# drdeford/FlipComplexityEmpirical

Hardware: AMD Instinct MI355X
Metric: flip steps/sec (whole node), 100×100 grid k=4 batched chains; % HBM peak (higher is better)
Workload: dtype int32

## Files before the change

### flipcomplexityempirical_amd/csrc/fw_grid16.hip

```cpp
#include <hip/hip_runtime.h>

#include <cstdio>
#include <cstdlib>

#include <algorithm>

#include "fw_device.h"
#include "fw_weights_bytes.h"
#include "fw_window_rows.h"

#ifdef FW_STAMPS
__device__ unsigned long long g_stamps[16];
__device__ unsigned long long g_unit_t[2 * 65536];
__device__ unsigned long long g_unit_hw[65536];
#define UNIT_TIME(u, e)                                                         \
  do {                                                                          \
    uint64_t t_;                                                                \
    asm volatile("s_memrealtime %0\n\ts_waitcnt lgkmcnt(0)" : "=s"(t_)::"memory"); \
    if (__lane_id() == 0 && (u) < 65536) {                                      \
      g_unit_t[2 * (u) + (e)] = t_;                                             \
      if ((e) == 0)                                                             \
        g_unit_hw[u] = (unsigned long long)__builtin_amdgcn_s_getreg((31 << 11) | 4) | \
                       ((unsigned long long)__builtin_amdgcn_s_getreg((31 << 11) | 20) << 32); \
    }                                                                           \
  } while (0)
#define STAMP_DECL uint64_t st_acc[16] = {}; uint64_t st_t0 = 0;
#define STAMP(i)                                              \
  do {                                                        \
    __builtin_amdgcn_sched_barrier(0);                        \
    uint64_t st_t1;                                           \
    asm volatile("s_memtime %0\n\ts_waitcnt lgkmcnt(0)" : "=s"(st_t1)::"memory"); \
    __builtin_amdgcn_sched_barrier(0);                        \
    if (i >= 0) st_acc[(i) < 0 ? 0 : (i)] += st_t1 - st_t0;   \
    st_t0 = st_t1;                                            \
  } while (0)
#define STAMP_FLUSH                                           \
  if (__lane_id() == 0)                                       \
    for (int i_ = 0; i_ < 16; ++i_) atomicAdd(&g_stamps[i_], (unsigned long long)st_acc[i_]);
#define STAMP_COUNT(i, v) st_acc[i] += (uint64_t)(v)
#else
#define STAMP_COUNT(i, v)
#define STAMP_DECL
#define STAMP(i)
#define STAMP_FLUSH
#define UNIT_TIME(u, e)
#endif

#include <cstddef>

static_assert(sizeof(fw_chain_stats) == 136, "fw_chain_stats layout");
static_assert(offsetof(fw_chain_stats, yields) == 88 && offsetof(fw_chain_stats, sum_invb) == 112 &&
                  offsetof(fw_chain_stats, cut) == 120 && offsetof(fw_chain_stats, npairs) == 128,
              "fw_chain_stats layout");

#define HIST_ADD(ptr, v) atomicAdd(ptr, v)

void* fw_grid16_pick_lean(int lb, int mode, int G, bool w4);
void* fw_grid16_pick_w2(int mode, int G, bool w4);

namespace {

constexpr int ROW = 16;
constexpr int MAX_NW = 4;
constexpr uint32_t SCR_BLOCK = 15;
constexpr int LDS_GUARD = 16;

struct Hood16 {
  int x;
  uint32_t lx;
  uint32_t bits;
  uint32_t cnt;
  bool has_v;
  int deg;
};

struct GDiv {
  uint32_t m, s;
  __device__ __forceinline__ int operator()(int x) const {
    return (int)(__umul24((uint32_t)x, m) >> s);
  }
};
__device__ __forceinline__ int mulW(int r, int W) { return (int)__umul24((uint32_t)r, (uint32_t)W); }

__device__ __forceinline__ uint32_t rowbits(uint64_t bal, int row) {
  return (uint32_t)(bal >> (row * ROW)) & 0xFFFFu;
}
__device__ __forceinline__ uint32_t row_scan(uint32_t x) {
  x += (uint32_t)__builtin_amdgcn_update_dpp(0, (int)x, 0x111, 0xF, 0xF, true);
  x += (uint32_t)__builtin_amdgcn_update_dpp(0, (int)x, 0x112, 0xF, 0xF, true);
  x += (uint32_t)__builtin_amdgcn_update_dpp(0, (int)x, 0x114, 0xF, 0xF, true);
  x += (uint32_t)__builtin_amdgcn_update_dpp(0, (int)x, 0x118, 0xF, 0xF, true);
  return x;
}
__device__ __forceinline__ uint32_t row_last(uint32_t x) {
  return (uint32_t)__builtin_amdgcn_update_dpp(0, (int)x, 0x15F, 0xF, 0xF, false);
}
__device__ __forceinline__ uint32_t row_sum(uint32_t x) { return row_last(row_scan(x)); }
__device__ __forceinline__ uint32_t row_first(uint32_t x) {
  return (uint32_t)__builtin_amdgcn_update_dpp(0, (int)x, 0x150, 0xF, 0xF, false);
}
__device__ __forceinline__ uint32_t row_shl1(uint32_t x) {
  return (uint32_t)__builtin_amdgcn_update_dpp(0, (int)x, 0x101, 0xF, 0xF, false);
}
__device__ __forceinline__ uint32_t row_pick(uint32_t x, int L, int q) {
  const int src = ((__lane_id() - q) + L) << 2;
  return (uint32_t)__builtin_amdgcn_ds_bpermute(src, (int)x);
}

template <int LB>
__device__ __forceinline__ uint32_t lab_window(const LDS uint8_t* lab, int x) {
  const int bit = (x - 1) * LB;
  const int wi = bit >> 5;
  const LDS uint32_t* w = reinterpret_cast<const LDS uint32_t*>(lab);
  const uint32_t lo0 = w[wi];
  const uint32_t lo = wi >= 0 ? lo0 : 0u;
  const uint32_t hi = w[wi + 1];
  const uint64_t both = ((uint64_t)hi << 32) | lo;
  return (uint32_t)(both >> (uint32_t)(bit - wi * 32)) & ((1u << (6 * LB)) - 1u);
}

template <int LB, int MODE>
__device__ __forceinline__ void weights4(const LDS uint8_t* lab, int x0, int W, int H, int n,
                                         GDiv gd, uint32_t& w4, uint32_t& cd4) {
  constexpr uint32_t M = (1u << LB) - 1u;
  w4 = 0;
  cd4 = 0;
  if (x0 >= n) return;
  const uint32_t own = lab_window<LB>(lab, x0);
  const uint32_t up = x0 + 3 - W >= 0 ? lab_window<LB>(lab, x0 - W) : 0u;
  const uint32_t dn = x0 + W < n ? lab_window<LB>(lab, x0 + W) : 0u;
  const int r0 = gd(x0);
  const int c0 = x0 - mulW(r0, W);
#pragma unroll
  for (int tt = 0; tt < 4; ++tt) {
    int ct = c0 + tt, rt = r0;
    if (ct >= W) {
      ct -= W;
      rt += 1;
    }
    const uint32_t lx = (own >> (LB * (tt + 1))) & M;
    const uint32_t ll = (own >> (LB * tt)) & M;
    const uint32_t lr = (own >> (LB * (tt + 2))) & M;
    const uint32_t lu = (up >> (LB * (tt + 1))) & M, ld = (dn >> (LB * (tt + 1))) & M;
    uint32_t bits = 0, cd = 0;
    if (rt > 0) { bits |= 1u << lu; cd += lu != lx; }
    if (ct > 0) { bits |= 1u << ll; cd += ll != lx; }
    if (ct < W - 1) { bits |= 1u << lr; cd += lr != lx; }
    if (rt < H - 1) { bits |= 1u << ld; cd += ld != lx; }
    uint32_t w = MODE == FW_PROPOSE_CUTEDGE ? cd : (uint32_t)__popc(bits & ~(1u << lx));
    if (x0 + tt >= n) w = cd = 0;
    w4 |= w << (8 * tt);
    cd4 |= cd << (8 * tt);
  }
}

__device__ __forceinline__ uint32_t bsum4(uint32_t v) {
  return (v & 0xFFu) + ((v >> 8) & 0xFFu) + ((v >> 16) & 0xFFu) + (v >> 24);
}

__device__ __forceinline__ uint32_t spread4(uint32_t u) {
  const uint32_t t = ((u << 12) | u) & 0x000F000Fu;
// ... 209 lines not shown
        else
          V |= nw;
      }
    }
  }
  if (verdict < 0) return -1;
  const uint32_t pc = (uint32_t)__popc(P);
  uint32_t dg = pc * (uint32_t)((r > 0) + (r < H - 1) + 2);
  if (c0 <= 0) dg -= (P >> (-c0)) & 1u;
  if (hi_n <= 32) dg -= (P >> (hi_n - 1)) & 1u;
  nodes = row_sum(pc);
  degs = row_sum(dg);
  return verdict;
}

__device__ __forceinline__ uint32_t lane_read(uint32_t x, int L) {
  return (uint32_t)__builtin_amdgcn_ds_bpermute(L << 2, (int)x);
}
template <int R>
__device__ __forceinline__ uint32_t grp_sum(uint32_t x, int gb, int q) {
  uint32_t t = 0;
#pragma unroll
  for (int s = 0; s < R; ++s) t += lane_read(x, gb + s * ROW + q);
  return t;
}
template <int R>
__device__ __forceinline__ uint64_t grp_sum64(uint64_t x, int gb, int q) {
  uint64_t t = 0;
#pragma unroll
  for (int s = 0; s < R; ++s)
    t += (uint64_t)lane_read((uint32_t)x, gb + s * ROW + q) |
         ((uint64_t)lane_read((uint32_t)(x >> 32), gb + s * ROW + q) << 32);
  return t;
}

__device__ __forceinline__ void scr_clear(LDS uint8_t* scr, int x) {
  __atomic_fetch_and(PK<4>::word(scr, x), ~(15u << PK<4>::shift(x)), __ATOMIC_RELAXED);
}

template <int LB>
__device__ bool grid_race(const LDS uint8_t* lab, LDS uint8_t* scr, LDS uint32_t* list,
                          GLB uint32_t* spill, int qcap, int W, int H, GDiv gd, int lane,
                          int v, uint32_t a, int m, int src, uint64_t cls, uint64_t& bfs_nodes,
                          uint64_t& bfs_deg) {
  using P = PK<LB>;
  using S = PK<4>;
  auto list_get = [&](int i) -> uint32_t {
    const uint32_t in_lds = list[i < qcap ? i : qcap - 1];
    uint32_t in_hbm = 0;
    if (i >= qcap) in_hbm = spill[i - qcap];
    return i < qcap ? in_lds : in_hbm;
  };
  auto list_put = [&](int i, uint32_t x) {
    if (i < qcap) list[i] = x;
    if (i >= qcap) spill[i - qcap] = x;
  };
  if (lane == 0) S::axor(scr, v, SCR_BLOCK);
  if (lane < m) {
    S::axor(scr, src, 1u + (uint32_t)lane);
    list_put(lane, (uint32_t)src);
  }
  lds_order();
  int nl = m, lb = 0, le = m;
  uint32_t my_deg = 0;
  int verdict = -1;
  for (;;) {
    uint64_t rep = ballot(lane < m && (__ffsll((unsigned long long)cls) - 1) == lane);
    if (__popcll(rep) == 1) {
      verdict = 1;
      break;
    }
    uint64_t pushed_src = 0;
    for (int base = lb; base < le; base += WAVE) {
      const int idx = base + lane;
      const bool act = idx < le;
      const int x = act ? (int)list_get(idx) : 0;
      const uint32_t o = act ? S::get(scr, x) - 1u : 0u;
      const int xr = gd(x);
      const int xc = x - mulW(xr, W);
      if (act) my_deg += (uint32_t)((xr > 0) + (xc > 0) + (xc < W - 1) + (xr < H - 1));
      bfs_nodes += (uint64_t)__popcll(ballot(act));
#pragma unroll
      for (int j = 0; j < 4; ++j) {
        int y = -1;
        if (act) {
          if (j == 0 && xr > 0) y = x - W;
          if (j == 1 && xc > 0) y = x - 1;
          if (j == 2 && xc < W - 1) y = x + 1;
          if (j == 3 && xr < H - 1) y = x + W;
        }
        bool push = false, req = false;
        uint32_t other = 0;
        if (y >= 0 && P::get(lab, y) == a) {
          const uint32_t got = S::claim(scr, y, 0u, 1u + o);
          if (got == 0u) {
            push = true;
          } else if (got - 1u < (uint32_t)m) {
            req = true;
            other = got - 1u;
          }
        }
        const uint64_t pm = ballot(push);
        if (push) list_put(nl + (int)mbcnt(pm), (uint32_t)y);
        nl += __popcll(pm);
        if (pm) {
          for (int si = 0; si < m; ++si)
            pushed_src |= ballot(push && o == (uint32_t)si) ? (1ull << si) : 0ull;
        }
        uint64_t rm = ballot(req && o != other);
        while (rm) {
          const int Lr = __ffsll((unsigned long long)rm) - 1;
          rm &= rm - 1;
          const int o1 = rdl((int32_t)o, Lr), o2 = rdl((int32_t)other, Lr);
          const uint64_t m1 = rdl64(cls, o1), m2 = rdl64(cls, o2);
          if (m1 != m2) {
            const uint64_t nm = m1 | m2;
            if (lane < m && ((nm >> lane) & 1ull)) cls = nm;
          }
        }
      }
      if (nl > qcap) __threadfence_block();
    }
    lds_order();
    lb = le;
    le = nl;
    rep = ballot(lane < m && (__ffsll((unsigned long long)cls) - 1) == lane);
    if (__popcll(rep) == 1) {
      verdict = 1;
      break;
    }
    const bool closed = lane < m && ((rep >> lane) & 1ull) && ((cls & pushed_src) == 0ull);
    if (ballot(closed)) {
      verdict = 0;
      break;
    }
  }
  bfs_deg += wave_sum(my_deg);
  for (int base = 0; base < nl; base += WAVE) {
    const int idx = base + lane;
    if (idx < nl) scr_clear(scr, (int)list_get(idx));
  }
  if (lane == 0) scr_clear(scr, v);
  lds_order();
  return verdict == 1;
}

template <int LB, int MODE, int PER, bool FULL, bool BIG, int R, bool W2 = false, bool W4 = false>
__device__ __forceinline__ void grid16_body(const FwRunParams& p) {
  static_assert(!W4 || LB == 2, "the width flag belongs to the SWAR weights");
  static_assert(PER % 2 == 0, "group sums are read as u16 pairs");
  static_assert(R == 1 || R == 2 || R == 4, "rows per chain");
  static_assert(R == 1 || (!FULL && !BIG), "speculation: lean small-grid kernels only");
  constexpr int CPW = 4 / R;
  extern __shared__ __align__(16) uint8_t smem[];
  __shared__ int32_t s_lock;
  using P = PK<LB>;
  const int lane = __lane_id(), row = lane >> 4, q = lane & 15;
  const int sx = row & (R - 1);
  const int grp = row / R;
  const int gb = grp * R * ROW;
  const bool owner = sx == 0;
  const int wv = (int)(threadIdx.x >> 6);
  const int W = (int)in_vgpr((uint32_t)p.g.gw), H = (int)in_vgpr((uint32_t)p.g.gh);
  const int n = (int)in_vgpr((uint32_t)p.g.n);
  const int D = (int)in_vgpr((uint32_t)p.g.maxdeg), G = (int)in_vgpr((uint32_t)p.G);
  const int k = (int)in_vgpr((uint32_t)p.k);
  LDS uint8_t* const sm = (LDS uint8_t*)smem;
  LDS uint8_t* const lab = sm + LDS_GUARD + (wv * CPW + grp) * p.slot_stride;
  LDS uint32_t* const gsum = reinterpret_cast<LDS uint32_t*>(lab + p.off_gsum);
  LDS uint32_t* const ssum = reinterpret_cast<LDS uint32_t*>(lab + p.off_ssum);
  LDS uint32_t* const lvl1 = BIG ? ssum : gsum;
  LDS uint8_t* const scr = sm + p.off_scr;
  LDS uint32_t* const list = reinterpret_cast<LDS uint32_t*>(sm + p.off_list16);
  GLB uint32_t* const spill = (GLB uint32_t*)(p.spill + (size_t)blockIdx.x * (size_t)n);
  const uint32_t key0 = (uint32_t)p.seed, key1 = (uint32_t)(p.seed >> 32);
  const int GW = (G + 1) >> 1;
  const int SG = (G + 15) >> 4;
  const bool maps_on = FULL && p.m_acc != nullptr;
  const int32_t pop_lo = (int32_t)in_vgpr((uint32_t)(int32_t)max(p.pop_lo, (int64_t)INT32_MIN));
  const int32_t pop_hi = (int32_t)in_vgpr((uint32_t)(int32_t)min(p.pop_hi, (int64_t)INT32_MAX));
  const GDiv gd{in_vgpr(p.g.gm24), in_vgpr(p.g.gs24)};
  const int32_t rule = FULL ? p.accept : FW_ACCEPT_CUT;
  int my_dr, my_dc;
  role_off(q <= 8 ? q : 0, my_dr, my_dc);
  if (LB == 2 && q >= 9 && q <= 12) {
    my_dr = q == 9 ? -2 : (q == 12 ? 2 : 0);
    my_dc = q == 10 ? -2 : (q == 11 ? 2 : 0);
  }
  const uint32_t nb_lanes = q == 0   ? 0x1Eu
                            : q == 1 ? (1u << 9) | (1u << 8) | (1u << 5)
                            : q == 2 ? (1u << 10) | (1u << 8) | (1u << 7)
                            : q == 3 ? (1u << 11) | (1u << 5) | (1u << 6)
                            : q == 4 ? (1u << 12) | (1u << 6) | (1u << 7)
                                     : 0u;
  auto divmod = [&](int x, int& r, int& c) {
    r = gd(x);
    c = x - mulW(r, W);
  };
  STAMP_DECL

  {
    LDS uint32_t* s32 = reinterpret_cast<LDS uint32_t*>(scr);
    for (int i = (int)threadIdx.x; i < p.scr_bytes / 4; i += (int)blockDim.x) s32[i] = 0u;
    if (threadIdx.x == 0) s_lock = 0;
  }
  __syncthreads();

  const int nq = (p.n_chains + CPW - 1) / CPW;
  for (;;) {
    int cb = 0;
    if (lane == 0) cb = atomicAdd(p.next_chain, 1);
    const int u = rdl(cb, 0);
    if (u >= nq * p.slices) break;
    const int seg = u / nq;
    const int quad = u - seg * nq;
    const uint32_t ustep = (uint32_t)(p.steps * (seg + 1) / p.slices - p.steps * seg / p.slices);
    if (seg > 0) {
      for (;;) {
        const int done =
            rfl(__hip_atomic_load(p.seg_done + quad, __ATOMIC_RELAXED, __HIP_MEMORY_SCOPE_AGENT));
        if (done >= seg) break;
        __builtin_amdgcn_s_sleep(2);
      }
      __builtin_amdgcn_fence(__ATOMIC_ACQUIRE, "agent");
    }
    UNIT_TIME(u, 0);
    const int cbase = quad * CPW;
    const int c = cbase + grp;
    const bool has = c < p.n_chains;
    const int cc = has ? c : cbase;
    const uint64_t gid = (uint64_t)(p.chain_id0 + c);
    const bool cached = p.gcache_ok != 0 || seg > 0;

    constexpr bool OPQ = R > 1 || MODE == FW_PROPOSE_CUTEDGE;
    int ql = q;
    if constexpr (OPQ) asm volatile("" : "+v"(ql));
    {
      const u32x4* src = reinterpret_cast<const u32x4*>(p.labels + (size_t)cc * p.lab_stride);
      LDS u32x4* dst = reinterpret_cast<LDS u32x4*>(lab);
      const int nv = cached ? p.lab_copy16 : p.lab_bytes / 16;
      for (int i = sx * ROW + ql; i < nv; i += R * ROW) dst[i] = src[i];
    }
    int32_t pops = ql < k ? (int32_t)p.pops[(size_t)cc * k + ql] : 0;
    double thr_l = FULL && ql < 2 * D + 1 ? p.thr[(size_t)cc * p.thr_stride + ql] : 0.0;
    uint64_t thr53_l = ql < 2 * D + 1 ? p.thr53[(size_t)cc * p.thr_stride + ql] : 0ull;
    fw_chain_stats* stp = p.stats + cc;
    const uint64_t acc0 = FULL && p.sched ? stp->accepts : 0ull;
    auto sched_row = [&](uint64_t nacc) {
      const int64_t t = (int64_t)(acc0 + nacc) + 1 - p.sched_t0;
      const int64_t r = t < 0 ? 0 : (t >= p.sched_rows ? p.sched_rows - 1 : t);
      if (q < 2 * D + 1) {
        thr_l = p.sched[r * (2 * D + 1) + q];
        thr53_l = p.sched53[r * (2 * D + 1) + q];
      }
    };
    if (FULL && p.sched) sched_row(0);
    uint64_t att0 = stp->attempts;
    const bool first = has && !stp->stuck && stp->yields == 0 && att0 == 0;
    uint32_t n_att = 0;
    const uint64_t yields0 = stp->yields;
    int32_t stuck = has ? stp->stuck : 1;
    uint32_t s_cut = 0, s_bn = 0;
    double sum_invb = stp->sum_invb;
    const bool waits_on = FULL && p.wsamp != nullptr;
    double wsum = waits_on ? p.wsamp[2 * (size_t)cc] : 0.0;
    double wcur = waits_on ? p.wsamp[2 * (size_t)cc + 1] : 0.0;
    uint32_t n_steps = 0, n_acc = 0, n_popf = 0, n_conf = 0, n_sdeg = 0, n_adeg = 0, n_bchg = 0;
    uint32_t retries = 0;
    uint64_t n_bfs = 0, n_bfsn = 0, n_bfsd = 0;
    uint32_t bpos_w = ROW * R;
    Pend pend = maps_on ? pend_load(p, cc) : Pend{-1, 0, 0u};
    int32_t bcnt = rule == FW_ACCEPT_BOUNDARY && ql < k ? p.bcnt[(size_t)cc * k + ql] : 0;
    lds_order();

    int32_t cut, bnodes, npairs;
    {
      uint32_t cut2 = 0, bn = 0, np = 0;
      for (int t2 = 0; t2 < (cached ? 0 : GW); ++t2) {
        uint32_t tot[2];
#pragma unroll
        for (int h = 0; h < 2; ++h) {
          uint32_t w4, cd4;
          weights4x<LB, MODE, true, true, W4>(lab, 2 * t2 + h, q, W, H, n, gd, w4, cd4);
          const uint32_t ws = bsum4m(w4);
          cut2 += bsum4m(cd4);
          bn += ((cd4 & 0xFFu) != 0) + ((cd4 & 0xFF00u) != 0) + ((cd4 & 0xFF0000u) != 0) +
                ((cd4 & 0xFF000000u) != 0);
          np += ws;
          tot[h] = row_sum(ws);
        }
        if (q == 0 && has) gsum[t2] = tot[0] | (tot[1] << 16);
      }
      if constexpr (BIG) {
        for (int t2 = GW + q; t2 < SG * 8; t2 += ROW)
          if (has) gsum[t2] = 0u;
        lds_order();
        for (int w2 = q; w2 < 8 * PER; w2 += ROW) {
          uint32_t s2[2] = {0u, 0u};
#pragma unroll
          for (int h = 0; h < 2; ++h) {
            const int sg = 2 * w2 + h;
            if (sg < SG)
              for (int i = 0; i < 8; ++i) {
                const uint32_t g2 = gsum[sg * 8 + i];
                s2[h] += (g2 & 0xFFFFu) + (g2 >> 16);
              }
          }
          if (has) ssum[w2] = s2[0] | (s2[1] << 16);
        }
      } else {
        for (int t2 = GW + q; t2 < 8 * PER; t2 += ROW)
          if (has) gsum[t2] = 0u;
      }
      if (cached) {
        cut = stp->cut;
        bnodes = stp->bnodes;
        npairs = stp->npairs;
      } else {
        cut = (int32_t)(row_sum(cut2) / 2);
        bnodes = (int32_t)row_sum(bn);
        npairs = (int32_t)row_sum(np);
      }
    }
    lds_order();
    double invb = p.g.invb[bnodes];

    const int RN = FULL ? p.ring_n : 0;
    auto ring_pair = [&]() -> int32_t {
      int f = -1, sc = -1;
      for (int b0 = 0; b0 < RN; b0 += ROW) {
        const int r = b0 + q;
        const int ri = r < RN ? r : 0;
        uint32_t m = rowbits(ballot(r < RN && P::get(lab, p.ring_u[ri]) != P::get(lab, p.ring_w[ri])),
                             row);
        if (m && f < 0) {
          f = b0 + __ffs(m) - 1;
          m &= m - 1;
        }
        if (m && sc < 0) sc = b0 + __ffs(m) - 1;
      }
      return sc >= 0 ? f * RN + sc : RN * RN;
    };
    int32_t rpair = RN && has ? ring_pair() : 0;
    uint32_t rrun = 0;

    uint32_t hc0 = 0, hc1 = 0, hb0 = 0, hb1 = 0;
    int32_t base_c = max(0, cut - 16), base_b = max(0, bnodes - 16);
    auto observe = [&](bool on) {
      if (!on) return;
      if (FULL) rrun += 1;
      if (waits_on) wsum += wcur;
      s_cut += (uint32_t)cut;
      s_bn += (uint32_t)bnodes;
      sum_invb += invb;
      int ic = cut - base_c;
      if (ic < 0 || ic >= 2 * ROW) {
        if (hc0) HIST_ADD(p.hist_cut + base_c + q, (unsigned long long)hc0);
        if (hc1) HIST_ADD(p.hist_cut + base_c + ROW + q, (unsigned long long)hc1);
        hc0 = hc1 = 0;
        base_c = max(0, cut - ROW);
        ic = cut - base_c;
      }
      hc0 += ic == q;
      hc1 += ic == q + ROW;
      int ib = bnodes - base_b;
      if (ib < 0 || ib >= 2 * ROW) {
        if (hb0) HIST_ADD(p.hist_b + base_b + q, (unsigned long long)hb0);
        if (hb1) HIST_ADD(p.hist_b + base_b + ROW + q, (unsigned long long)hb1);
        hb0 = hb1 = 0;
        base_b = max(0, bnodes - ROW);
        ib = bnodes - base_b;
      }
      hb0 += ib == q;
      hb1 += ib == q + ROW;
    };
    if (waits_on && first) wcur = wait_draw(p.seed, FW_WAIT_T0, gid, p.wlp[bnodes]);
    observe(first && owner);

    U4 pb = {0u, 0u, 0u, 0u};
    int bpos = ROW;
    uint32_t w2[PER / 2];
    auto read_lvl1 = [&]() {
#pragma unroll
      for (int t = 0; t < PER / 2; ++t) w2[t] = lvl1[q * (PER / 2) + t];
    };
    read_lvl1();

    const bool unit_pop = !FULL || p.g.pop == nullptr;
    const uint32_t psh = (uint32_t)p.prio_shift;
    const uint32_t pstep = ustep >= (2u << psh) ? ustep >> psh : 2u;
    uint32_t pnext = pstep, plev = 0;
    if (psh == 3u && (__builtin_amdgcn_s_getreg((3 << 11) | 4) & 1u) == 0u) plev = 1;
    if (plev == 0) __builtin_amdgcn_s_setprio(3);
    else __builtin_amdgcn_s_setprio(2);
    for (;;) {
      STAMP(-1);
      if (!stuck && (retries >= (uint32_t)p.max_retries || npairs == 0)) stuck = 1;
      const bool act = has && !stuck && n_steps < ustep;
      if (ballot(act) == 0ull) break;
      if (rfl(n_steps) >= pnext) {
        pnext += pstep;
        plev = (plev + 1u) & 3u;
        if (plev == 0) __builtin_amdgcn_s_setprio(3);
        else if (plev == 1) __builtin_amdgcn_s_setprio(2);
        else if (plev == 2) __builtin_amdgcn_s_setprio(1);
        else __builtin_amdgcn_s_setprio(0);
      }

      U4 x;
      if constexpr (R == 1) {
        if (bpos == ROW) {
          if (n_sdeg >= p.fold_at || (s_cut | s_bn) >= p.fold_at) {
            if (q == 0 && has) {
              stp->pop_fail += n_popf;
              stp->contig_fail += n_conf;
              stp->sum_deg += n_sdeg;
              stp->sum_cut += s_cut;
              stp->sum_bnodes += s_bn;
            }
            att0 += n_att;
            n_att = n_popf = n_conf = n_sdeg = 0;
            s_cut = s_bn = 0;
          }
          const uint64_t t = att0 + (uint64_t)(n_att + (uint32_t)q);
          pb = philox((uint32_t)t, (uint32_t)(t >> 32), (uint32_t)gid, (uint32_t)(gid >> 32),
                      in_vgpr(key0), in_vgpr(key1));
          bpos = 0;
        }
        x = U4{row_first(pb.x0), row_first(pb.x1), row_first(pb.x2), row_first(pb.x3)};
        pb = U4{row_shl1(pb.x0), row_shl1(pb.x1), row_shl1(pb.x2), row_shl1(pb.x3)};
        ++bpos;
        n_att += act ? 1u : 0u;
      } else {
        if (bpos_w > (uint32_t)(ROW * R - R)) {
          const uint32_t s_any = lane_read(s_cut | s_bn, gb + q);
          if (4u * n_att >= p.fold_at || s_any >= p.fold_at) {
            const uint32_t f0 = grp_sum<R>(n_popf, gb, q), f1 = grp_sum<R>(n_conf, gb, q);
            const uint32_t f2 = grp_sum<R>(n_sdeg, gb, q);
            if (q == 0 && owner && has) {
              stp->pop_fail += f0;
              stp->contig_fail += f1;
              stp->sum_deg += f2;
              stp->sum_cut += s_cut;
              stp->sum_bnodes += s_bn;
            }
            att0 += n_att;
            n_att = n_popf = n_conf = n_sdeg = 0;
            s_cut = s_bn = 0;
          }
          const uint64_t t = att0 + (uint64_t)(n_att + (uint32_t)(sx * ROW + q));
          pb = philox((uint32_t)t, (uint32_t)(t >> 32), (uint32_t)gid, (uint32_t)(gid >> 32),
                      in_vgpr(key0), in_vgpr(key1));
          bpos_w = 0;
        }
        const int srcl = gb + (int)bpos_w + sx;
        x = U4{lane_read(pb.x0, srcl), lane_read(pb.x1, srcl), lane_read(pb.x2, srcl),
               lane_read(pb.x3, srcl)};
      }
      const uint32_t r = scale64(x.x0, x.x1, (uint32_t)(npairs > 0 ? npairs : 1));

      STAMP(0);
      uint32_t s = 0;
#pragma unroll
      for (int t = 0; t < PER / 2; ++t) s += (w2[t] & 0xFFFFu) + (w2[t] >> 16);
      uint32_t pp[PER / 2];
      {
        uint32_t base = 0;
#pragma unroll
        for (int t = 0; t < PER / 2; ++t) {
          pp[t] = __umul24(base, 0x10001u) + (w2[t] + (w2[t] << 16));
          base = pp[t] >> 16;
        }
      }
      const uint32_t incl = row_scan(s);
      const uint32_t rb1 = rowbits(ballot(incl > r), row);
      const int Lw = __ffs(rb1) - 1;
      const uint32_t rl = r - (incl - s);
      typedef uint16_t u16x2 __attribute__((ext_vector_type(2)));
      const u16x2 rl2 = __builtin_bit_cast(u16x2, __umul24(rl & 0xFFFFu, 0x10001u));
      u16x2 mn = {0xFFFFu, 0xFFFFu}, wraps = {0u, 0u};
#pragma unroll
      for (int t = 0; t < PER / 2; ++t) {
        const u16x2 e = rl2 - __builtin_bit_cast(u16x2, pp[t]);
        mn = __builtin_elementwise_min(mn, e);
        wraps += e >> (uint16_t)15;
      }
      const uint32_t rem = min(rl, (uint32_t)min(mn.x, mn.y));
      const int tfu = PER - (int)wraps.x - (int)wraps.y;
      const int tf = min(tfu, PER - 1);
      const uint32_t pk1 = row_pick(((uint32_t)(q * PER + tf) << 16) | (rem & 0xFFFFu), Lw, q);
      int gi;
      uint32_t r1;
      uint32_t rbg = 1u;
      if constexpr (BIG) {
        const int sgi = min((int)(pk1 >> 16), SG - 1);
        const uint32_t r1s = pk1 & 0xFFFFu;
        const uint32_t g2 = gsum[sgi * 8 + (q >> 1)];
        const uint32_t gv = (q & 1) ? (g2 >> 16) : (g2 & 0xFFFFu);
        const uint32_t incg = row_scan(gv);
        rbg = rowbits(ballot(incg > r1s), row);
        const int Lg = __ffs(rbg) - 1;
        const uint32_t pkg =
            row_pick(((uint32_t)(sgi * 16 + q) << 16) | ((r1s - (incg - gv)) & 0xFFFFu), Lg, q);
        gi = min((int)(pkg >> 16), G - 1);
        r1 = pkg & 0xFFFFu;
      } else {
        gi = min((int)(pk1 >> 16), G - 1);
        r1 = pk1 & 0xFFFFu;
      }

      STAMP(1);
      uint32_t w4, cd4;
      weights4x<LB, MODE, false, !W2, W4>(lab, gi, q, W, H, n, gd, w4, cd4);
      const uint32_t pref1 = w4 + (w4 << 8);
      const uint32_t pref = pref1 + (pref1 << 16);
      const uint32_t ws = pref >> 24;
      const uint32_t incl2 = row_scan(ws);
      const uint32_t rb2 = rowbits(ballot(incl2 > r1), row);
      const int L2 = __ffs(rb2) - 1;
      const uint32_t r2 = min(r1 - (incl2 - ws), 127u);
      const uint32_t gt = ((pref | 0x80808080u) - __builtin_amdgcn_perm(0u, r2 + 1u, 0u)) & 0x80808080u;
      const int t2 = gt ? (__ffs(gt) - 1) >> 3 : 3;
      const uint32_t bef2 = t2 ? (pref >> (8 * t2 - 8)) & 0xFFu : 0u;
      const uint32_t pk2 = row_pick(((uint32_t)(q * 4 + t2) << 16) | ((r2 - bef2) & 0xFFFFu), L2, q);
      const int v = min(gi * 64 + (int)(pk2 >> 16), n - 1);
      const uint32_t j = pk2 & 0xFFFFu;
      if (R == 1 && act && (rb1 == 0 || rb2 == 0 || rbg == 0)) stuck = 2;
      const bool go = act && rb1 != 0 && rb2 != 0 && rbg != 0;

      STAMP(2);
      int vr, vc;
      divmod(v, vr, vc);
      const int dv = (vr > 0) + (vc > 0) + (vc < W - 1) + (vr < H - 1);
      Hood16 h;
      h.x = -1;
      h.lx = NOLAB;
      h.bits = 0;
      h.cnt = 0;
      h.has_v = false;
      h.deg = 0;
      if constexpr (LB == 2) {
        const int xr = vr + my_dr, xc = vc + my_dc;
        const bool inb = (q <= 12) & ((uint32_t)xr < (uint32_t)H) & ((uint32_t)xc < (uint32_t)W);
        const int xx = mulW(xr, W) + xc;
        const uint32_t l0 = P::get(lab, inb ? xx : v);
        h.x = inb ? xx : -1;
        h.lx = inb ? l0 : NOLAB;
        const uint32_t m0 = rowbits(ballot(h.lx == 0u), row) & nb_lanes;
        const uint32_t m1 = rowbits(ballot(h.lx == 1u), row) & nb_lanes;
        const uint32_t m2 = rowbits(ballot(h.lx == 2u), row) & nb_lanes;
        const uint32_t m3 = rowbits(ballot(h.lx == 3u), row) & nb_lanes;
        h.bits = (m0 ? 1u : 0u) | (m1 ? 2u : 0u) | (m2 ? 4u : 0u) | (m3 ? 8u : 0u);
        if constexpr (MODE == FW_PROPOSE_CUTEDGE) {
          const uint32_t same = h.lx == 0u ? m0 : h.lx == 1u ? m1 : h.lx == 2u ? m2 : m3;
          h.cnt = (uint32_t)__popc(m0 | m1 | m2 | m3) - (uint32_t)__popc(same);
          h.deg = q == 0 ? (int)h.cnt + (int)__popc(same) : 0;
        }
        h.has_v = q >= 1 && q <= 4 && inb;
        if (!(inb && q <= 4)) {
          h.bits = 0;
          h.cnt = 0;
        }
      } else {
        const int xr = vr + my_dr, xc = vc + my_dc;
        if (q <= 8 && xr >= 0 && xr < H && xc >= 0 && xc < W) {
          h.x = xr * W + xc;
          h.lx = P::get(lab, h.x);
          if (q <= 4) {
            h.deg = (xr > 0) + (xc > 0) + (xc < W - 1) + (xr < H - 1);
            const int vslot = 4 - q;
#pragma unroll
            for (int jj = 0; jj < 4; ++jj) {
              int y = -1;
              if (jj == 0 && xr > 0) y = h.x - W;
              if (jj == 1 && xc > 0) y = h.x - 1;
              if (jj == 2 && xc < W - 1) y = h.x + 1;
              if (jj == 3 && xr < H - 1) y = h.x + W;
              if (y < 0) continue;
              if (q > 0 && jj == vslot) {
                h.has_v = true;
                continue;
              }
              const uint32_t ly = P::get(lab, y);
              h.bits |= 1u << ly;
              h.cnt += ly != h.lx;
            }
          }
        }
      }
      const uint32_t a = row_first(h.lx);
      const bool isnb = q >= 1 && q <= 4 && h.x >= 0;
      uint32_t d;
      if constexpr (MODE == FW_PROPOSE_CUTEDGE) {
        const uint32_t cm = rowbits(ballot(isnb && h.lx != a), row) >> 1;
        uint32_t mm = cm;
        for (uint32_t t = 0; t < j && t < 4; ++t) mm &= mm - 1;
        const int Lc = __ffs(mm);
        d = row_pick(h.lx, Lc, q);
      } else {
        uint32_t mask;
        if constexpr (LB == 2) {
          mask = row_first(h.bits) & ~(1u << a);
        } else {
          uint32_t fb = (isnb && h.lx != a) ? (1u << h.lx) : 0u;
          fb |= (uint32_t)__builtin_amdgcn_update_dpp(0, (int)fb, 0x111, 0xF, 0xF, true);
          fb |= (uint32_t)__builtin_amdgcn_update_dpp(0, (int)fb, 0x112, 0xF, 0xF, true);
          fb |= (uint32_t)__builtin_amdgcn_update_dpp(0, (int)fb, 0x114, 0xF, 0xF, true);
          mask = (uint32_t)__builtin_amdgcn_update_dpp(0, (int)fb, 0x154, 0xF, 0xF, false);
        }
        uint32_t mm = mask;
        if constexpr (LB == 2) {
          const uint32_t m1 = mm & (mm - 1u), m2 = m1 & (m1 - 1u);
          mm = j == 0u ? mm : (j == 1u ? m1 : m2);
        } else {
          for (uint32_t t = 0; t < j && t < 15; ++t) mm &= mm - 1;
        }
        d = (uint32_t)(__ffs(mm) - 1);
      }
      const uint32_t amb = rowbits(ballot(isnb && h.lx == a), row) >> 1;
      const int m = __popc(amb);
      const int nbd = __popc(rowbits(ballot(isnb && h.lx == d), row) >> 1);
      const int dcut = m - nbd;

// ... 72 lines not shown
        uint32_t vt = win_touch(fx, q) | (win_miss(fx, ex4) ? 1u : 0u);
        vt |= (uint32_t)__builtin_amdgcn_update_dpp(0, (int)vt, 0x111, 0xF, 0xF, true);
        vt |= (uint32_t)__builtin_amdgcn_update_dpp(0, (int)vt, 0x112, 0xF, 0xF, true);
        vt |= (uint32_t)__builtin_amdgcn_update_dpp(0, (int)vt, 0x114, 0xF, 0xF, true);
        vt = (uint32_t)__builtin_amdgcn_update_dpp(0, (int)vt, 0x156, 0xF, 0xF, false);
        const int wvd = win_verdict((vt & 1u) != 0u, vt, ex4);
        STAMP_COUNT(12, 1);
        STAMP_COUNT(13, nflood);
        if (need & (wvd >= 0)) {
          contig = wvd == 1;
          need = false;
        }
      }
      STAMP(7);
      if (BIG && !p.no_bb && !p.no_rowbb && ballot(need)) {
        uint32_t bn16 = 0, bd16 = 0;
        const int vb = grid_race_bb_row<LB>(lab, n, W, H, q, row, need, vr, vc, a, amb,
                                            (uint32_t)(lNE | (lES << 1) | (lSW << 2) | (lWN << 3)),
                                            bn16, bd16);
        if (need && vb >= 0) {
          contig = vb == 1;
          need = false;
          count_search(bn16, bd16);
        }
      }
      uint64_t rows_need = ballot(q == 0 && need);
      bool locked = false;
      while (rows_need) {
        const int L0 = __ffsll((unsigned long long)rows_need) - 1;
        rows_need &= rows_need - 1;
        const int rr = L0 >> 4;
        if constexpr (R > 1) {
          if (rr % R) {
            const uint64_t sure = ballot(q == 0 && go && pop_ok && contig && wacc);
            const uint32_t before = (uint32_t)((1u << (rr % R)) - 1u) << (rr - rr % R);
            uint32_t rows_sure = 0;
#pragma unroll
            for (int r4 = 0; r4 < 4; ++r4) rows_sure |= ((sure >> (16 * r4)) & 1u) << r4;
            if (rows_sure & before) continue;
          }
        }
        const uint32_t aa = rdl(a, L0);
        const uint32_t am4 = rdl(amb, L0);
        const uint32_t lk = rdl((uint32_t)(lNE | (lES << 1) | (lSW << 2) | (lWN << 3)), L0);
        uint64_t bn = 0, bd = 0;
        int verdict = -1;
        if (!p.no_bb)
          verdict = grid_race_bb<LB>(sm + LDS_GUARD + (wv * CPW + rr / R) * p.slot_stride, n, W, H,
                                    lane, rdl(vr, L0), rdl(vc, L0), aa, am4, lk, bn, bd);
        if (verdict >= 0) {
          if (row == rr) {
            contig = verdict == 1;
            count_search(bn, bd);
          }
          continue;
        }
        if (!locked) {
          if (lane == 0) {
            int expect = 0;
            while (!__hip_atomic_compare_exchange_strong(&s_lock, &expect, 1, __ATOMIC_ACQUIRE,
                                                         __ATOMIC_RELAXED,
                                                         __HIP_MEMORY_SCOPE_WORKGROUP)) {
              expect = 0;
              __builtin_amdgcn_s_sleep(1);
            }
          }
          lds_order();
          locked = true;
        }
        const int vv = rdl(v, L0);
        const int mr = __popc(am4);
        int srcn = -1;
        uint32_t mm = am4;
        for (int i = 0; i < mr; ++i) {
          const int bit = __ffs(mm) - 1;
          mm &= mm - 1;
          const int val = rdl(h.x, L0 + 1 + bit);
          if (lane == i) srcn = val;
        }
        uint64_t cls = lane < mr ? (1ull << lane) : 0ull;
        auto sx = [&](int b) { return __popc(am4 & ((1u << b) - 1u)); };
        auto merge = [&](int s1, int s2) {
          const uint64_t nm = rdl64(cls, s1) | rdl64(cls, s2);
          if (lane < mr && ((nm >> lane) & 1ull)) cls = nm;
        };
        if (lk & 1) merge(sx(0), sx(2));
        if (lk & 2) merge(sx(2), sx(3));
        if (lk & 4) merge(sx(3), sx(1));
        if (lk & 8) merge(sx(1), sx(0));
        const bool ok = grid_race<LB>(sm + LDS_GUARD + (wv * CPW + rr / R) * p.slot_stride, scr, list, spill,
                                      p.qcap16, W, H, gd, lane, vv, aa, mr, srcn, cls, bn,
                                      bd);
        if (row == rr) {
          contig = ok;
          count_search(bn, bd);
        }
      }
      if (locked && lane == 0)
        __hip_atomic_store(&s_lock, 0, __ATOMIC_RELEASE, __HIP_MEMORY_SCOPE_WORKGROUP);

      STAMP(4);
      const bool valid = go && pop_ok && contig;
      if constexpr (R > 1) {
        const bool accepted = valid && wacc;
        const uint64_t b_go = ballot(q == 0 && go), b_val = ballot(q == 0 && valid);
        const uint64_t b_acc = ballot(q == 0 && accepted);
        uint32_t cons = 0, kold = 0, ns = n_steps, rt = retries;
        int fpos = -1;
        bool stop = !act;
#pragma unroll
        for (int s2 = 0; s2 < R; ++s2) {
          const int L = gb + s2 * ROW;
          const bool g2 = (b_go >> L) & 1ull, v2 = (b_val >> L) & 1ull, a2 = (b_acc >> L) & 1ull;
          if (!stop && !g2) {
            stuck = 2;
            stop = true;
          }
          if (!stop) {
            cons = (uint32_t)s2 + 1u;
            if (v2) {
              ns += 1u;
              rt = 0u;
              if (a2) {
                fpos = s2;
                stop = true;
              } else {
                kold += 1u;
              }
              if (ns >= ustep) stop = true;
            } else {
              rt += 1u;
              if (rt >= (uint32_t)p.max_retries) stop = true;
            }
          }
        }
        if (sx < (int)cons) {
          n_sdeg += (uint32_t)dv;
          if (!pop_ok) n_popf += 1;
          else if (!contig) n_conf += 1;
          n_bfs += it_bfs;
          n_bfsn += it_bfsn;
          n_bfsd += it_bfsd;
        }
        n_steps = ns;
        retries = rt;
        n_att += cons;
        bpos_w += cons;
        const bool commit_me = sx == fpos;
        if (commit_me) {
          n_acc += 1;
          n_adeg += (uint32_t)dv;
          n_bchg += (uint32_t)(plus + minus);
          if (q == 0) P::axor(lab, v, a ^ d);
          if (mine && wn != wo) lds_add(gsum + (h.x >> 7), (wn - wo) << (16 * ((h.x >> 6) & 1)));
        }
        lds_order();
        read_lvl1();
        uint32_t dl = commit_me && mine ? wn - wo : 0u;
        dl += (uint32_t)__builtin_amdgcn_update_dpp(0, (int)dl, 0x111, 0xF, 0xF, true);
        dl += (uint32_t)__builtin_amdgcn_update_dpp(0, (int)dl, 0x112, 0xF, 0xF, true);
        dl += (uint32_t)__builtin_amdgcn_update_dpp(0, (int)dl, 0x114, 0xF, 0xF, true);
        const int dnp = (int)(uint32_t)__builtin_amdgcn_update_dpp(0, (int)dl, 0x154, 0xF, 0xF, false);
        const int fsrc = gb + (fpos < 0 ? 0 : fpos) * ROW + q;
        const uint32_t pk = (uint32_t)(dcut + 8) | ((uint32_t)plus << 4) | ((uint32_t)minus << 8) |
                            (a << 12) | (d << 16) | ((uint32_t)(dnp + 64) << 20);
        const uint32_t pkf = lane_read(pk, fsrc);
        const uint64_t ib = (uint64_t)__double_as_longlong(invb_new);
        const uint32_t ibl = lane_read((uint32_t)ib, fsrc), ibh = lane_read((uint32_t)(ib >> 32), fsrc);
        for (uint32_t i = 0; i < kold; ++i) observe(owner);
        if (fpos >= 0) {
          npairs += (int)((pkf >> 20) & 127u) - 64;
          cut += (int)(pkf & 15u) - 8;
          bnodes += (int)((pkf >> 4) & 15u) - (int)((pkf >> 8) & 15u);
          invb = __longlong_as_double((long long)(((uint64_t)ibh << 32) | ibl));
          if ((uint32_t)q == ((pkf >> 12) & 15u)) pops -= 1;
          if ((uint32_t)q == ((pkf >> 16) & 15u)) pops += 1;
          observe(owner);
        }
        STAMP(5);
        continue;
      }
      if (go) {
        n_sdeg += (uint32_t)dv;
        if (!pop_ok) n_popf += 1;
        else if (!contig) n_conf += 1;
        retries = valid ? 0u : retries + 1u;
      }
      bool accepted;
      if (rule == FW_ACCEPT_BOUNDARY) {
        const int32_t fv = p.flags[v] ? 1 : 0;
        const int32_t cnt = bcnt - ((uint32_t)q == a ? fv : 0) + ((uint32_t)q == d ? fv : 0);
        accepted = valid && __popc(rowbits(ballot(q < k && cnt > 0), row)) >= 2;
      } else {
        bool acc_l;
        if (rule == FW_ACCEPT_BRATIO) {
          const double bound = thr_l * ((double)(bnodes + plus - minus) / (double)bnodes);
          acc_l = u53(x.x2, x.x3) < bound;
        } else {
          acc_l = (((uint64_t)(x.x2 >> 5) << 26) | (uint64_t)(x.x3 >> 6)) < thr53_l;
        }
        accepted = valid & (((rowbits(ballot(acc_l), row) >> (dcut + D)) & 1u) != 0u);
      }
      STAMP(8);
      if (FULL && p.trace != nullptr && valid && q == 0)
        p.trace[(size_t)c * p.steps + n_steps] = accepted ? v * 64 + (int)d : -1;
      n_steps += valid ? 1u : 0u;
      if (maps_on && accepted) {
        const int64_t t = (int64_t)(yields0 + (n_steps - 1u) + (first ? 1u : 0u));
        if (q >= 1 && q <= 4 && h.x >= 0 && (h.lx == a || h.lx == d)) {
          const int e = q == 1   ? grid_eid_down(vr - 1, vc, W, H)
                        : q == 2 ? grid_eid_right(vr, vc - 1, W, H)
                        : q == 3 ? grid_eid_right(vr, vc, W, H)
                                 : grid_eid_down(vr, vc, W, H);
          map_edge(p, c, e, h.lx == a, t);
        }
        if (q == 0) map_run_end(p, c, pend, t);
        pend = Pend{v, (int32_t)d, (uint32_t)t};
      }

      if (accepted) {
        if (q == 0) P::axor(lab, v, a ^ d);
        if (mine && wn != wo) {
          lds_add(gsum + (h.x >> 7), (wn - wo) << (16 * ((h.x >> 6) & 1)));
          if (BIG) lds_add(ssum + (h.x >> 11), (wn - wo) << (16 * ((h.x >> 10) & 1)));
        }
      }
      lds_order();
      read_lvl1();
      uint32_t dl = accepted && mine ? wn - wo : 0u;
      dl += (uint32_t)__builtin_amdgcn_update_dpp(0, (int)dl, 0x111, 0xF, 0xF, true);
      dl += (uint32_t)__builtin_amdgcn_update_dpp(0, (int)dl, 0x112, 0xF, 0xF, true);
      dl += (uint32_t)__builtin_amdgcn_update_dpp(0, (int)dl, 0x114, 0xF, 0xF, true);
      const int dnp = (int)(uint32_t)__builtin_amdgcn_update_dpp(0, (int)dl, 0x154, 0xF, 0xF, false);
      if (FULL && RN && accepted && p.ring_node[v]) {
        const int32_t np2 = ring_pair();
        if (np2 != rpair) {
          if (q == 0 && rrun) atomicAdd(p.hist_ring + rpair, (unsigned long long)rrun);
          rrun = 0;
          rpair = np2;
        }
      }
      STAMP(9);
      asm volatile("" ::"v"(invb_new));
      invb = accepted ? invb_new : invb;
      if (accepted) {
        n_acc += 1;
        if (FULL && p.sched) sched_row(n_acc);
        n_adeg += (uint32_t)dv;
        npairs += dnp;
        cut += dcut;
        bnodes += plus - minus;
        n_bchg += (uint32_t)(plus + minus);
        if ((uint32_t)q == a) pops -= pv;
        if ((uint32_t)q == d) pops += pv;
        if (rule == FW_ACCEPT_BOUNDARY && p.flags[v]) {
          if ((uint32_t)q == a) bcnt -= 1;
          if ((uint32_t)q == d) bcnt += 1;
        }
        if (waits_on) wcur = wait_draw(p.seed, att0 + (uint64_t)(n_att - 1u), gid, p.wlp[bnodes]);
      }
      observe(valid);
      STAMP(5);
    }

    STAMP(6);
    if constexpr (R > 1) {
      n_popf = grp_sum<R>(n_popf, gb, q);
      n_conf = grp_sum<R>(n_conf, gb, q);
      n_sdeg = grp_sum<R>(n_sdeg, gb, q);
      n_acc = grp_sum<R>(n_acc, gb, q);
      n_adeg = grp_sum<R>(n_adeg, gb, q);
      n_bchg = grp_sum<R>(n_bchg, gb, q);
      n_bfs = grp_sum64<R>(n_bfs, gb, q);
      n_bfsn = grp_sum64<R>(n_bfsn, gb, q);
      n_bfsd = grp_sum64<R>(n_bfsd, gb, q);
    }
    if (has && owner) {
      if (hc0) HIST_ADD(p.hist_cut + base_c + q, (unsigned long long)hc0);
      if (hc1) HIST_ADD(p.hist_cut + base_c + ROW + q, (unsigned long long)hc1);
      if (hb0) HIST_ADD(p.hist_b + base_b + q, (unsigned long long)hb0);
      if (hb1) HIST_ADD(p.hist_b + base_b + ROW + q, (unsigned long long)hb1);
      if (FULL && RN && q == 0 && rrun) atomicAdd(p.hist_ring + rpair, (unsigned long long)rrun);
      int qw = q;
      if constexpr (OPQ) asm volatile("" : "+v"(qw));
      u32x4* dst = reinterpret_cast<u32x4*>(p.labels + (size_t)c * p.lab_stride);
      const LDS u32x4* src = reinterpret_cast<const LDS u32x4*>(lab);
      for (int i = qw; i < p.lab_copy16; i += ROW) dst[i] = src[i];
      if (qw < k) p.pops[(size_t)c * k + qw] = (int64_t)pops;
      if (qw < k && rule == FW_ACCEPT_BOUNDARY) p.bcnt[(size_t)c * k + qw] = bcnt;
      if (q == 0 && maps_on) pend_store(p, c, pend);
      if (q == 0 && waits_on) {
        p.wsamp[2 * (size_t)c] = wsum;
        p.wsamp[2 * (size_t)c + 1] = wcur;
      }
      if (q <= 8) {
        int qr = qw;
        if constexpr (!OPQ) asm volatile("" : "+v"(qr));
        uint64_t* rec = reinterpret_cast<uint64_t*>(stp) + 2 * qr;
        const uint64_t o0 = rec[0];
        const uint64_t o1 = qr < 8 ? rec[1] : 0ull;
        const uint64_t yinc = (uint64_t)n_steps + (first ? 1u : 0u);
        uint64_t w0, w1;
        switch (q) {
          case 0: w0 = att0 + n_att; w1 = o1 + n_steps; break;
          case 1: w0 = o0 + n_acc; w1 = o1 + n_popf; break;
          case 2: w0 = o0 + n_conf; w1 = o1 + n_bfs; break;
          case 3: w0 = o0 + n_bfsn; w1 = o1 + n_bfsd; break;
          case 4: w0 = o0 + n_sdeg; w1 = o1 + n_adeg; break;
          case 5: w0 = o0 + n_bchg; w1 = o1 + yinc; break;
          case 6: w0 = o0 + s_cut; w1 = o1 + s_bn; break;
          case 7:
            w0 = (uint64_t)__double_as_longlong(sum_invb);
            w1 = (uint64_t)(uint32_t)cut | ((uint64_t)(uint32_t)bnodes << 32);
            break;
          default: w0 = (uint64_t)(uint32_t)npairs | ((uint64_t)(uint32_t)stuck << 32); w1 = 0;
        }
        if (qr < 8) {
          typedef uint64_t u64x2 __attribute__((ext_vector_type(2)));
          *reinterpret_cast<u64x2*>(rec) = u64x2{w0, w1};
        } else {
          rec[0] = w0;
        }
      }
    }
    lds_order();
    UNIT_TIME(u, 1);
    if (seg + 1 < p.slices) {
      __builtin_amdgcn_fence(__ATOMIC_RELEASE, "agent");
      __hip_atomic_store(p.seg_done + quad, seg + 1, __ATOMIC_RELAXED, __HIP_MEMORY_SCOPE_AGENT);
    }
  }
  STAMP_FLUSH
}

template <int LB, int MODE, int PER, bool FULL, bool BIG, bool W4 = false>
__global__ __launch_bounds__(64 * MAX_NW) __attribute__((amdgpu_waves_per_eu(3))) void fw_grid16_kernel(FwRunParams p) {
  static_assert(!FULL, "FULL instantiations: fw_grid16_full_kernel");
  grid16_body<LB, MODE, PER, FULL, BIG, 1, false, W4>(p);
}
template <int LB, int MODE, int PER, bool FULL, bool BIG>
__global__ __launch_bounds__(64 * MAX_NW) void fw_grid16_full_kernel(FwRunParams p) {
  grid16_body<LB, MODE, PER, true, BIG, 1>(p);
}
template <int LB, int MODE, int PER, bool W4>
__global__ __launch_bounds__(64 * MAX_NW) void fw_grid16_w2_kernel(FwRunParams p) {
  grid16_body<LB, MODE, PER, false, false, 1, true, W4>(p);
}

#ifndef FW_SPEC_WPE
#define FW_SPEC_WPE 3
#endif
template <int LB, int MODE, int PER, int R>
__global__ __launch_bounds__(64 * MAX_NW) __attribute__((amdgpu_waves_per_eu(FW_SPEC_WPE))) void
fw_grid16_spec_kernel(FwRunParams p) {
  grid16_body<LB, MODE, PER, false, false, R>(p);
}

int per16(int G) { return G <= 16 * 2 ? 2 : G <= 16 * 4 ? 4 : G <= 16 * 10 ? 10 : 16; }
int per16_big(int G) { return (G + 15) / 16 <= 32 ? 2 : 4; }
bool is_big(int G) { return G > 16 * 16; }

template <int LB, int MODE, int PER, bool FULL, bool BIG, bool W4 = false>
void* k16() {
  if constexpr (FULL)
    return reinterpret_cast<void*>(&fw_grid16_full_kernel<LB, MODE, PER, true, BIG>);
  else
    return reinterpret_cast<void*>(&fw_grid16_kernel<LB, MODE, PER, false, BIG, W4>);
}

template <int LB, int MODE, bool W4>
void* pick16_small_lean_w(int G) {
  switch (per16(G)) {
    case 2: return k16<LB, MODE, 2, false, false, W4>();
    case 4: return k16<LB, MODE, 4, false, false, W4>();
    case 10: return k16<LB, MODE, 10, false, false, W4>();
    default: return k16<LB, MODE, 16, false, false, W4>();
  }
}
template <int LB, int MODE>
void* pick16_small_lean(int G, bool w4) {
  if constexpr (LB == 2) {
    if (w4) return pick16_small_lean_w<LB, MODE, true>(G);
  }
  return pick16_small_lean_w<LB, MODE, false>(G);
}

template <int LB, int MODE, bool FULL>
void* pick16(int G, bool w4) {
  if (is_big(G)) {
    if constexpr (LB == 4) {
      return nullptr;
    } else {
      return per16_big(G) == 2
                 ? k16<LB, MODE, 2, FULL, true>()
                 : k16<LB, MODE, 4, FULL, true>();
    }
  }
  if constexpr (LB == 3) {
    return nullptr;
  } else if constexpr (FULL) {
    switch (per16(G)) {
      case 2: return k16<LB, MODE, 2, true, false>();
      case 4: return k16<LB, MODE, 4, true, false>();
      case 10: return k16<LB, MODE, 10, true, false>();
      default: return k16<LB, MODE, 16, true, false>();
    }
  } else {
#if defined(FW_STAMPS)
    return pick16_small_lean<LB, MODE>(G, w4);
#else
    return fw_grid16_pick_lean(LB, MODE, G, w4);
#endif
  }
}

template <int MODE, bool W4>
void* pick16_w2(int G) {
  if (is_big(G)) return nullptr;
  switch (per16(G)) {
    case 2: return reinterpret_cast<void*>(&fw_grid16_w2_kernel<2, MODE, 2, W4>);
    case 4: return reinterpret_cast<void*>(&fw_grid16_w2_kernel<2, MODE, 4, W4>);
    case 10: return reinterpret_cast<void*>(&fw_grid16_w2_kernel<2, MODE, 10, W4>);
    default: return reinterpret_cast<void*>(&fw_grid16_w2_kernel<2, MODE, 16, W4>);
  }
}

template <int LB, int MODE, int R>
void* pick16_spec(int G) {
  if (is_big(G) || LB == 3) return nullptr;
  switch (per16(G)) {
// ... 266 lines not shown
```

Baseline: 4.644 billion.

## Store level-1 weight sums as in-lane prefix sums to skip per-step scan

For small non-W2 kernels, the level-1 group-sum array in LDS now holds per-lane inclusive prefix sums instead of raw pair sums. Each step can read the lane total and prefixes directly, with no per-step summation and prefix loop. Weight updates now add the delta to every word from the changed position to the end of the lane's span, which means several LDS atomics instead of one. The array is converted back to raw sums before the final write-out.

After: 4.655 billion, median of 6. Within noise of the previous version (+0.2%).

```diff
diff --git a/flipcomplexityempirical_amd/csrc/fw_grid16.hip b/flipcomplexityempirical_amd/csrc/fw_grid16.hip
--- a/flipcomplexityempirical_amd/csrc/fw_grid16.hip
+++ b/flipcomplexityempirical_amd/csrc/fw_grid16.hip
@@ -7,6 +7,7 @@
 
 #include "fw_device.h"
 #include "fw_weights_bytes.h"
+#include "fw_lvl1_prefix.h"
 #include "fw_window_rows.h"
 
 #ifdef FW_STAMPS
@@ -522,6 +523,7 @@
   static_assert(R == 1 || R == 2 || R == 4, "rows per chain");
   static_assert(R == 1 || (!FULL && !BIG), "speculation: lean small-grid kernels only");
   constexpr int CPW = 4 / R;
+  constexpr bool L1P = !BIG && !W2;
   extern __shared__ __align__(16) uint8_t smem[];
   __shared__ int32_t s_lock;
   using P = PK<LB>;
@@ -693,6 +695,17 @@
       }
     }
     lds_order();
+    if constexpr (L1P) {
+      if (owner) {
+        uint32_t base = 0;
+#pragma unroll
+        for (int t = 0; t < PER / 2; ++t) {
+          LDS uint32_t* const wp = gsum + q * (PER / 2) + t;
+          *wp = l1_prefix_word(*wp, base);
+        }
+      }
+      lds_order();
+    }
     double invb = p.g.invb[bnodes];
 
     const int RN = FULL ? p.ring_n : 0;
@@ -749,12 +762,26 @@
 
     U4 pb = {0u, 0u, 0u, 0u};
     int bpos = ROW;
-    uint32_t w2[PER / 2];
+    uint32_t pp[PER / 2];
     auto read_lvl1 = [&]() {
 #pragma unroll
-      for (int t = 0; t < PER / 2; ++t) w2[t] = lvl1[q * (PER / 2) + t];
+      for (int t = 0; t < PER / 2; ++t) pp[t] = lvl1[q * (PER / 2) + t];
     };
     read_lvl1();
+    auto lvl1_commit = [&](int x, uint32_t dlt) {
+      if constexpr (!L1P) {
+        lds_add(gsum + (x >> 7), dlt << (16 * ((x >> 6) & 1)));
+        if (BIG) lds_add(ssum + (x >> 11), dlt << (16 * ((x >> 10) & 1)));
+      } else {
+        int jw, cnt;
+        l1_commit_span<PER / 2>(x, jw, cnt);
+        LDS uint32_t* const wp = gsum + jw;
+        lds_add(wp, l1_commit_addend(dlt, x, 0));
+#pragma unroll
+        for (int t = 1; t < PER / 2; ++t)
+          if (t < cnt) lds_add(wp + t, l1_commit_addend(dlt, x, t));
+      }
+    };
 
     const bool unit_pop = !FULL || p.g.pop == nullptr;
     const uint32_t psh = (uint32_t)p.prio_shift;
@@ -830,15 +857,17 @@
       const uint32_t r = scale64(x.x0, x.x1, (uint32_t)(npairs > 0 ? npairs : 1));
 
       STAMP(0);
-      uint32_t s = 0;
-#pragma unroll
-      for (int t = 0; t < PER / 2; ++t) s += (w2[t] & 0xFFFFu) + (w2[t] >> 16);
-      uint32_t pp[PER / 2];
-      {
+      uint32_t s;
+      if constexpr (L1P) {
+        s = pp[PER / 2 - 1] >> 16;
+      } else {
+        s = 0;
+#pragma unroll
+        for (int t = 0; t < PER / 2; ++t) s += (pp[t] & 0xFFFFu) + (pp[t] >> 16);
         uint32_t base = 0;
 #pragma unroll
         for (int t = 0; t < PER / 2; ++t) {
-          pp[t] = __umul24(base, 0x10001u) + (w2[t] + (w2[t] << 16));
+          pp[t] = __umul24(base, 0x10001u) + (pp[t] + (pp[t] << 16));
           base = pp[t] >> 16;
         }
       }
@@ -1217,7 +1246,7 @@
           n_adeg += (uint32_t)dv;
           n_bchg += (uint32_t)(plus + minus);
           if (q == 0) P::axor(lab, v, a ^ d);
-          if (mine && wn != wo) lds_add(gsum + (h.x >> 7), (wn - wo) << (16 * ((h.x >> 6) & 1)));
+          if (mine && wn != wo) lvl1_commit(h.x, wn - wo);
         }
         lds_order();
         read_lvl1();
@@ -1285,10 +1314,7 @@
 
       if (accepted) {
         if (q == 0) P::axor(lab, v, a ^ d);
-        if (mine && wn != wo) {
-          lds_add(gsum + (h.x >> 7), (wn - wo) << (16 * ((h.x >> 6) & 1)));
-          if (BIG) lds_add(ssum + (h.x >> 11), (wn - wo) << (16 * ((h.x >> 10) & 1)));
-        }
+        if (mine && wn != wo) lvl1_commit(h.x, wn - wo);
       }
       lds_order();
       read_lvl1();
@@ -1341,6 +1367,15 @@
       n_bfsd = grp_sum64<R>(n_bfsd, gb, q);
     }
     if (has && owner) {
+      if constexpr (L1P) {
+        uint32_t base = 0;
+#pragma unroll
+        for (int t = 0; t < PER / 2; ++t) {
+          LDS uint32_t* const wp = gsum + q * (PER / 2) + t;
+          *wp = l1_sums_word(*wp, base);
+        }
+        lds_order();
+      }
       if (hc0) HIST_ADD(p.hist_cut + base_c + q, (unsigned long long)hc0);
       if (hc1) HIST_ADD(p.hist_cut + base_c + ROW + q, (unsigned long long)hc1);
       if (hb0) HIST_ADD(p.hist_b + base_b + q, (unsigned long long)hb0);
diff --git a/flipcomplexityempirical_amd/csrc/fw_lvl1_prefix.h b/flipcomplexityempirical_amd/csrc/fw_lvl1_prefix.h
--- /dev/null
+++ b/flipcomplexityempirical_amd/csrc/fw_lvl1_prefix.h
@@ -0,0 +1,36 @@
+#pragma once
+#include <stdint.h>
+
+#if defined(__HIPCC__) || defined(__CUDACC__)
+#define FW_L1_FN __host__ __device__ inline
+#else
+#define FW_L1_FN inline
+#endif
+
+FW_L1_FN uint32_t l1_prefix_word(uint32_t sums, uint32_t& base) {
+  const uint32_t t = base + sums;
+  const uint32_t pp = t + (t << 16);
+  base = pp >> 16;
+  return pp;
+}
+
+FW_L1_FN uint32_t l1_sums_word(uint32_t prefixes, uint32_t& base) {
+  const uint32_t lo = prefixes & 0xFFFFu, hi = prefixes >> 16;
+  const uint32_t sums = ((lo - base) & 0xFFFFu) | ((hi - lo) << 16);
+  base = hi;
+  return sums;
+}
+
+template <int PER2>
+FW_L1_FN void l1_commit_span(int x, int& jw, int& cnt) {
+  static_assert(PER2 == 1 || PER2 == 2 || PER2 == 5 || PER2 == 8, "PER in {2, 4, 10, 16}");
+  constexpr uint32_t M = (1024u + PER2 - 1) / PER2;
+  jw = x >> 7;
+  const int lane = (int)(((uint32_t)jw * M) >> 10);
+  cnt = (lane + 1) * PER2 - jw;
+}
+
+FW_L1_FN uint32_t l1_commit_addend(uint32_t delta, int x, int t) {
+  const uint32_t both = delta + (delta << 16);
+  return t == 0 && ((x >> 6) & 1) ? delta << 16 : both;
+}
```
